# williamedwards/autompc

Measured on AMD Instinct MI355X. Metric: MPC solves/sec (MPPI, n_samples x horizon rollouts + update per solve), higher is better.
Workload: dtype f64; 1 GPU; c3: HalfCheetah (17-dim state, 6-dim ctrl), MLP 2x256, MPPI 4096 samples x 30 horizon; random-weight model, QuadCost Q=I R=0.01I F=I, sigma=1 lmda=1, 1 independent solve(s) per step per GPU, noise=device; n_samples=4096, horizon=30, state_dim=17, ctrl_dim=6, parallelism=independent solves per GPU (dp1)

## Files before the change

autompc_amd/csrc/mlp_tile.hpp:

```cpp
#pragma once
#include <hip/hip_runtime.h>

#include <type_traits>

#include "probe.hpp"

namespace ampc {

constexpr int kMaxHidden = 4;
constexpr int kMaxWaves = 8;

typedef double d4 __attribute__((ext_vector_type(4)));
typedef float f4 __attribute__((ext_vector_type(4)));

template <typename T> struct Acc;
template <> struct Acc<double> { using type = d4; };
template <> struct Acc<float> { using type = f4; };

__device__ __forceinline__ d4 mfma16(double a, double b, d4 c) {
  if constexpr (Probe::no_mfma) { c[0] += a * b; return c; }
  else return __builtin_amdgcn_mfma_f64_16x16x4f64(a, b, c, 0, 0, 0);
}
__device__ __forceinline__ f4 mfma16(float a, float b, f4 c) {
  if constexpr (Probe::no_mfma) { c[0] += a * b; return c; }
// ... 376 lines not shown
        __builtin_amdgcn_sched_group_barrier(0x020, SG, 0);
        __builtin_amdgcn_sched_group_barrier(0x100, 2 * MT, 0);
#pragma unroll
        for (int i = 0; i < SG / 2; ++i) {
          __builtin_amdgcn_sched_group_barrier(0x008, 2 * MT * NT, 0);
          __builtin_amdgcn_sched_group_barrier(0x100, MT, 0);
        }
      } else if constexpr (sizeof(T) == 4 && (Probe::f32_ahead > 0 || Probe::f32_fine > 0)) {
        constexpr int AH = Probe::f32_ahead > 0 ? Probe::f32_ahead : 2;
        __builtin_amdgcn_sched_group_barrier(0x100, AH * MT, 0);
        if constexpr (Probe::f32_fine == 1) {
#pragma unroll
          for (int i = 0; i < SG; ++i) {
            __builtin_amdgcn_sched_group_barrier(0x008, MT * NT, 0);
            if (i + AH < SG) __builtin_amdgcn_sched_group_barrier(0x100, MT, 0);
            __builtin_amdgcn_sched_group_barrier(0x020, 1, 0);
          }
        } else if constexpr (Probe::f32_fine == 2) {
          constexpr int H1 = (MT * NT + 1) / 2, H2 = MT * NT - H1;
#pragma unroll
          for (int i = 0; i < SG; ++i) {
            __builtin_amdgcn_sched_group_barrier(0x008, H1, 0);
            if (i + AH < SG) __builtin_amdgcn_sched_group_barrier(0x100, MT, 0);
            if (H2 > 0) __builtin_amdgcn_sched_group_barrier(0x008, H2, 0);
            __builtin_amdgcn_sched_group_barrier(0x020, 1, 0);
          }
        } else if constexpr (Probe::f32_fine == 3) {
#pragma unroll
          for (int i = 0; i < SG; ++i) {
            __builtin_amdgcn_sched_group_barrier(0x008, MT * NT, 0);
            __builtin_amdgcn_sched_group_barrier(0x020, 1, 0);
            if (i + AH < SG) __builtin_amdgcn_sched_group_barrier(0x100, MT, 0);
          }
        } else {
#pragma unroll
          for (int i = 0; i < SG / 2; ++i) {
            __builtin_amdgcn_sched_group_barrier(0x008, 2 * MT * NT, 0);
            if (2 * i + AH < SG) __builtin_amdgcn_sched_group_barrier(0x100, MT, 0);
            if (2 * i + AH + 1 < SG) __builtin_amdgcn_sched_group_barrier(0x100, MT, 0);
            __builtin_amdgcn_sched_group_barrier(0x020, 2, 0);
          }
        }
      } else if (REG0 && sgi < FS) {
#pragma unroll
        for (int i = 0; i < SG / 2; ++i) {
          __builtin_amdgcn_sched_group_barrier(0x008, 2 * MT * NT, 0);
          __builtin_amdgcn_sched_group_barrier(0x020, 2, 0);
        }
      } else {
        __builtin_amdgcn_sched_group_barrier(0x100, 2 * MT, 0);
#pragma unroll
        for (int i = 0; i < SG / 2; ++i) {
          __builtin_amdgcn_sched_group_barrier(0x008, 2 * MT * NT, 0);
          __builtin_amdgcn_sched_group_barrier(0x100, MT, 0);
          __builtin_amdgcn_sched_group_barrier(0x020, 2, 0);
        }
      }
    }
    if (OWN && sgi == FS - 1) {
      lds_barrier();
      mid();
    }
    if constexpr (Probe::valu_pad) {
      if (KS >= 16 && sgi >= 2 && sgi < 10) {
        int padv = lane;
#pragma unroll
        for (int pi = 0; pi < 8; ++pi) asm volatile("v_add_u32 %0, %0, 1" : "+v"(padv));
        asm volatile("" :: "v"(padv));
      }
    }
    if constexpr (Probe::valu_pad64) {
      if (KS >= 16 && sgi >= 2 && sgi < 10) {
        double padd = (double)lane;
#pragma unroll
        for (int pi = 0; pi < 8; ++pi) asm volatile("v_add_f64 %0, %0, 1.0" : "+v"(padd));
        asm volatile("" :: "v"(padd));
      }
    }
  }
}


template <typename T, int NT, int MT, int W, bool DERIV = false, int LEAN = 0, typename SH = DynShape,
          bool WIDE = false, bool PINNED = false, bool BIAS0K = false>
struct TileNet {
  using acc_t = typename Acc<T>::type;
  static constexpr int M = 16 * MT;
  static constexpr int HP = 16 * NT * W;
  static constexpr int KSH = HP / 4;
  static constexpr int KSW = KSH / W;
  static constexpr int KS0MAX = 12;
  static constexpr int GH = 8;
  static constexpr int NOMAX = WIDE ? 4 : 2;
  static constexpr bool OWN = (16 * NT == 4 * GH) && (((KSH / GH) & (KSH / GH - 1)) == 0);
  static constexpr bool PIN = PINNED && SH::kStatic && sizeof(T) == 8;
  static constexpr bool CHAIN = PIN && MT == 1 && !DERIV && !WIDE && LEAN == 0;
  static constexpr int BR = (CHAIN && W == 8) ? 4 : 1;
  static constexpr bool CHAIN_BIAS_LDS = CHAIN && BR == 1;
  static constexpr bool BIAS0_IN_K = BIAS0K && CHAIN && !Probe::no_res0 && SH::k1p <= 24 && SH::nx + SH::nu < SH::k1p;

  static constexpr int KS0RES = sizeof(T) == 4 ? KS0MAX : 6;
  T pf0[KS0RES][NT];
  __device__ __forceinline__ static bool resident0(const MlpDev<T>& m) {
    return !Probe::no_res0 && LEAN < 2 && (sizeof(T) == 4 || MT == 1) && m.k1p <= 4 * KS0RES;
  }

  __device__ __forceinline__ static unsigned slice0(const MlpDev<T>& m, int w) {
    return (unsigned)(m.W(0) - m.WB()) + (unsigned)w * (unsigned)(m.k1p / 4) * 64u * NT;
  }
  __device__ __forceinline__ static unsigned slice_h(const MlpDev<T>& m, int l, int w) {
    return (unsigned)(m.W(l) - m.WB()) + (unsigned)w * (unsigned)KSH * 64u * NT;
  }
  rsrc_t wr;
  template <int KS> __device__ __forceinline__ const T (&first0() const)[KS][NT] {
    return reinterpret_cast<const T(&)[KS][NT]>(pf0);
  }
  template <int KS> __device__ __forceinline__ T (&first0())[KS][NT] {
    return reinterpret_cast<T(&)[KS][NT]>(pf0);
  }

  static constexpr bool RESIDENT_OUT = WIDE || (LEAN < 2 && !(MT == 4 && sizeof(T) == 8));
  T wout[KSW][NOMAX];

  __device__ __forceinline__ static void load_out(const MlpDev<T>& m, int w, int lane,
                                                  T (&dst)[KSW][NOMAX]) {
    if constexpr (WIDE) {
      const int tiles = m.nxp / 16;
      const T* wl = m.W(m.n_hidden) + ((size_t)w * KSW * 64 + lane) * tiles;
#pragma unroll
      for (int ks = 0; ks < KSW; ++ks)
#pragma unroll
        for (int n = 0; n < NOMAX; ++n) dst[ks][n] = n < tiles ? wl[(size_t)ks * 64 * tiles + n] : T(0);
    } else if (m.nxp == 16) {
      const T* wl = m.W(m.n_hidden) + ((size_t)w * KSW * 64 + lane);
#pragma unroll
      for (int ks = 0; ks < KSW; ++ks) { dst[ks][0] = wl[ks * 64]; dst[ks][1] = T(0); }
    } else {
      const T* wl = m.W(m.n_hidden) + ((size_t)w * KSW * 64 + lane) * 2;
#pragma unroll
      for (int ks = 0; ks < KSW; ++ks) { const vec_t<T, 2> v = *reinterpret_cast<const vec_t<T, 2>*>(wl + ks * 128); dst[ks][0] = v[0]; dst[ks][1] = v[1]; }
      if (m.tail4) {
        const T* wt = m.WT() + ((size_t)w * KSW * 64 + lane);
#pragma unroll
        for (int ks = 0; ks < KSW; ++ks) dst[ks][1] = wt[ks * 64];
      }
    }
  }

  static constexpr bool RESIDENT_BIAS = LEAN < 1 && (MT == 1);
  static constexpr int kResBias = 2;
  T bias_r[kResBias][NT][BR];
  T pfn[GH][NT];
  ProbeWave<Probe::wave_time> probe;

  lds_ptr<const T> bq_;
  static constexpr int RS = sizeof(T) == 8 ? 4 : 1;
  static constexpr int NGH = KSH / GH;
  lds_ptr<T> ep_[2][4];
  lds_ptr<const T> rd_[2][NGH];
  lds_ptr<const T> ro_;
  lds_ptr<const T> x0_;
  lds_ptr<T> pp_, pt_;
  int w_;

  __device__ __forceinline__ void pin(const MlpDev<T>& m_in, const TileLds& L_in, T* lds) {
    if constexpr (PIN) {
      const MlpDev<T> m = SH::template fold<T>(m_in);
      const TileLds L = SH::template fold_lds<T, M, W>(L_in);
      const int lane = threadIdx.x & 63;
      const int w = w_ = __builtin_amdgcn_readfirstlane(threadIdx.x >> 6);
      const int i = lane & 15, q = lane >> 4;
      const int as = L.act_stride;
      const bool pingpong = L.act2 != L.act;
#pragma unroll
      for (int b = 0; b < 2; ++b) {
        T* buf = lds + (b ? L.act2 : L.act);
        const bool read = b == 0 ? m.n_hidden > 1 : (pingpong && m.n_hidden > 2);
        const bool written = CHAIN ? read : (b == 0 || pingpong);
#pragma unroll
        for (int r = 0; r < 4; ++r) {
          if constexpr (CHAIN)
            ep_[b][r] = (written && r == 0) ? lds_pin(buf + i * as + 16 * NT * w + q) : lds_ptr<T>(nullptr);
// ... 234 lines not shown
    };
    auto epilogue_chain = [&](int l, acc_t (&acc)[MT][NT], int db, bool store) {
      switch (m.act) {
        case 0: chain_k(l, acc, db, store, std::integral_constant<int, 0>{}); break;
        case 1: chain_k(l, acc, db, store, std::integral_constant<int, 1>{}); break;
        case 2: chain_k(l, acc, db, store, std::integral_constant<int, 2>{}); break;
        case 4: chain_k(l, acc, db, store, std::integral_constant<int, 4>{}); break;
        default: chain_k(l, acc, db, store, std::integral_constant<int, 3>{}); break;
      }
    };

    bool side_done = false;
    {
      acc_t acc[MT][NT];
#pragma unroll
      for (int mt = 0; mt < MT; ++mt)
#pragma unroll
        for (int nt = 0; nt < NT; ++nt) acc[mt][nt] = acc_t{0, 0, 0, 0};
      const unsigned wl = slice0(m, w);
      const T* A = lds + L.xu;
      if (m.n_hidden == 1) prefetch_next(1);
      if (resident0(m)) {
        const auto arow0 = [&] {
          if constexpr (PIN) return x0_;
          else return A + i * L.xu_stride + q;
        }();
        switch (m.k1p) {
          case 8: layer0_resident<2>(arow0, L.xu_stride, acc); break;
          case 16: layer0_resident<4>(arow0, L.xu_stride, acc); break;
          case 24: layer0_resident<6>(arow0, L.xu_stride, acc); break;
          default:
            if constexpr (KS0RES >= 12) {
              switch (m.k1p) {
                case 32: layer0_resident<8>(arow0, L.xu_stride, acc); break;
                case 40: layer0_resident<10>(arow0, L.xu_stride, acc); break;
                default: layer0_resident<12>(arow0, L.xu_stride, acc); break;
              }
            }
            break;
        }
      } else {
        auto layer0_streamed = [&](auto ks) {
          layer_mma_static<T, NT, MT, decltype(ks)::value, 2, false, false, 2, false, CHAIN>(
              A, L.xu_stride, wr, wl, lane, first0<2>(), acc);
        };
        switch (m.k1p) {
          case 8: layer0_streamed(std::integral_constant<int, 2>{}); break;
          case 16: layer0_streamed(std::integral_constant<int, 4>{}); break;
          case 24: layer0_streamed(std::integral_constant<int, 6>{}); break;
          case 32: layer0_streamed(std::integral_constant<int, 8>{}); break;
          case 40: layer0_streamed(std::integral_constant<int, 10>{}); break;
          case 48: layer0_streamed(std::integral_constant<int, 12>{}); break;
          default:
            if constexpr (WIDE) {
              switch (m.k1p) {
                case 56: layer0_streamed(std::integral_constant<int, 14>{}); break;
                case 64: layer0_streamed(std::integral_constant<int, 16>{}); break;
                case 72: layer0_streamed(std::integral_constant<int, 18>{}); break;
                default: layer0_streamed(std::integral_constant<int, 20>{}); break;
              }
            } else {
              layer0_streamed(std::integral_constant<int, 12>{});
            }
            break;
        }
      }
      AMPC_MARK(2);
      if constexpr (CHAIN) epilogue_chain(0, acc, 0, m.n_hidden > 1);
      else epilogue(0, acc, act, 0);
    }
    if (!OWN && m.n_hidden > 1) lds_barrier();
    AMPC_MARK(3);

    for (int l = 1; l < m.n_hidden; ++l) {
      acc_t acc[MT][NT];
#pragma unroll
      for (int mt = 0; mt < MT; ++mt)
#pragma unroll
        for (int nt = 0; nt < NT; ++nt) {
          acc[mt][nt] = acc_t{0, 0, 0, 0};
        }
      constexpr int SGH = (sizeof(T) == 8 && !Probe::sg8) ? GH / 2 : GH;
      auto mid = [&] {
        if (!Probe::side_late && l == 1) { side(); side_done = true; }
      };
      auto pinned_group = [&](int g) {
        if constexpr (OWN) return cur ? rd_[1][g] : rd_[0][g];
        else return (cur ? rd_[1][0] : rd_[0][0]) + 4 * GH * g;
      };
      if constexpr (CHAIN && OWN)
        layer_mma_static<T, NT, MT, KSH, GH, (W == 8), OWN, SGH, true, true>(
            act, as, wr, slice_h(m, l, w), lane, pfn, acc, w, mid, pinned_group,
            [&](int kk) { return own[kk >> 2][kk & 3]; });
      else if constexpr (PIN)
        layer_mma_static<T, NT, MT, KSH, GH, (W == 8), OWN, SGH, true, CHAIN>(
            act, as, wr, slice_h(m, l, w), lane, pfn, acc, w, mid, pinned_group);
      else
        layer_mma_static<T, NT, MT, KSH, GH, (W == 8), OWN, SGH, true>(
            act, as, wr, slice_h(m, l, w), lane, pfn, acc, w, mid);
      AMPC_MARK(4);
      prefetch_next(l + 1);
      const bool stores = !CHAIN || l + 1 < m.n_hidden;
      if (!pingpong && stores) lds_barrier();
      AMPC_MARK(5);
      if constexpr (CHAIN) epilogue_chain(l, acc, pingpong ? cur ^ 1 : 0, stores);
      else epilogue(l, acc, act_other, pingpong ? cur ^ 1 : 0);
      if (!OWN && l + 1 < m.n_hidden) lds_barrier();
      AMPC_MARK(6);
      { T* tmp = act; act = act_other; act_other = tmp; }
      if (pingpong) cur ^= 1;
    }

    acc_t oacc[MT][NOMAX];
    T tacc[MT];
#pragma unroll
    for (int mt = 0; mt < MT; ++mt) {
      tacc[mt] = T(0);
#pragma unroll
      for (int n = 0; n < NOMAX; ++n) oacc[mt][n] = acc_t{0, 0, 0, 0};
    }
    {
      const auto arow = [&] {
        if constexpr (PIN) return ro_;
        else return static_cast<const T*>(act) + act_row<T>(i) * as + q + 4 * w * KSW;
      }();
      auto afrag = [&](int mt, int ks) -> T {
        if constexpr (CHAIN) return own[ks >> 2][ks & 3];
        else return arow[mt * 16 * as + 4 * ks];
      };
      if constexpr (WIDE) {
#pragma unroll
        for (int ks = 0; ks < KSW; ++ks)
#pragma unroll
          for (int mt = 0; mt < MT; ++mt) {
            const T a = afrag(mt, ks);
#pragma unroll
            for (int n = 0; n < NOMAX; ++n)
              if (n < no) oacc[mt][n] = mfma16_x<kRealOut>(a, wo(ks, n), oacc[mt][n]);
          }
      } else if (no == 1) {
#pragma unroll
        for (int ks = 0; ks < KSW; ++ks)
#pragma unroll
          for (int mt = 0; mt < MT; ++mt)
            oacc[mt][0] = mfma16_x<kRealOut>(afrag(mt, ks), wo(ks, 0), oacc[mt][0]);
      } else if (m.tail4) {
#pragma unroll
        for (int ks = 0; ks < KSW; ++ks)
#pragma unroll
          for (int mt = 0; mt < MT; ++mt) {
            const T a = afrag(mt, ks);
            oacc[mt][0] = mfma16_x<kRealOut>(a, wo(ks, 0), oacc[mt][0]);
            tacc[mt] = kRealOut ? mfma4(a, wo(ks, 1), tacc[mt]) : tacc[mt] + a * wo(ks, 1);
          }
      } else {
#pragma unroll
        for (int ks = 0; ks < KSW; ++ks)
#pragma unroll
          for (int mt = 0; mt < MT; ++mt) {
            const T a = afrag(mt, ks);
            oacc[mt][0] = mfma16_x<kRealOut>(a, wo(ks, 0), oacc[mt][0]);
            oacc[mt][1] = mfma16_x<kRealOut>(a, wo(ks, 1), oacc[mt][1]);
          }
      }
    }
    AMPC_MARK(7);
    prefetch0(m);
    if (m.n_hidden > 1) prefetch_next(1);
    if (!side_done) {
      if (m.n_hidden == 1) lds_barrier();
      side();
    }
    if (L.part_alias) lds_barrier();
    AMPC_MARK(8);
    const int ps = part_stride((int)sizeof(T), m.nxp);
    T* part = lds + L.part + w * M * ps;
    const int nfull = m.tail4 ? 1 : no;
#pragma unroll
    for (int mt = 0; mt < MT; ++mt) {
#pragma unroll
      for (int n = 0; n < NOMAX; ++n)
        if (n < nfull) {
#pragma unroll
          for (int r = 0; r < 4; ++r) {
            if constexpr (PIN) {
              pp_[(16 * mt + RS * r) * ps + 16 * n] = oacc[mt][n][r];
            } else {
              const int row = 16 * mt + acc_row<T>(q, r);
              part[row * ps + 16 * n + i] = oacc[mt][n][r];
            }
          }
        }
      if (m.tail4) {
        if constexpr (PIN) pt_[16 * mt * ps] = tacc[mt];
        else part[(16 * mt + tail_row(lane)) * ps + 16 + tail_col(lane)] = tacc[mt];
      }
    }
    AMPC_MARK(13);
    lds_barrier();
    AMPC_MARK(9);
  }

  __device__ __forceinline__ static T output(const MlpDev<T>& m_in, const TileLds& L_in, const T* lds,
                                             int row, int col) {
    const MlpDev<T> m = SH::template fold<T>(m_in);
    const TileLds L = SH::template fold_lds<T, M, W>(L_in);
    const int ps = part_stride((int)sizeof(T), m.nxp);
    const T* p = lds + L.part + row * ps + col;
    T y = lds[L.bias + m.n_hidden * m.hpad + col];
#pragma unroll
    for (int w = 0; w < W; ++w) y += p[w * M * ps];
    return y;
  }
};

template <typename T>
__device__ __forceinline__ T quad_rows(const T* __restrict__ Mx, const T* __restrict__ v,
                                       const T* __restrict__ g, int n, int r, int tps, bool diag) {
  T acc = T(0);
  if (diag) {
    for (int i = r; i < n; i += tps) {
      const T d = v[i] - (g ? g[i] : T(0));
      acc += Mx[i * n + i] * d * d;
    }
  } else {
    for (int i = r; i < n; i += tps) {
      T s = T(0);
      for (int j = 0; j < n; ++j) s += Mx[i * n + j] * (v[j] - (g ? g[j] : T(0)));
      acc += (v[i] - (g ? g[i] : T(0))) * s;
    }
  }
  return acc;
}

template <typename T>
__device__ __forceinline__ T affine_rows(const T* __restrict__ lin, const T* __restrict__ v,
                                         const T* __restrict__ g, int n, int r, int tps, T c) {
  T acc = r == 0 ? c : T(0);
  for (int i = r; i < n; i += tps) acc += lin[i] * (v[i] - g[i]);
  return acc;
}

constexpr int kMaxInd = 8;
__host__ __device__ constexpr int ind_stride(int no) { return 2 * no + 2; }
template <typename T> __device__ __forceinline__ bool ind_entry(int kind, T x, T a, T b) {
  if (kind == 1) { const T d = x - a; return d > b || -d > b; }
  return x < a || x > b;
}
template <typename T> __device__ __forceinline__ bool ind_void(int kind, T x, T b) {
  return kind == 1 && x != x && b < T(INFINITY);
}
template <typename T>
__device__ __forceinline__ T indicator_rows(const T* __restrict__ tab, int n_ind, const T* __restrict__ v, int vs,
                                            int no, int r, int tps) {
  T acc = T(0);
  const int lane = threadIdx.x & 63;
  for (int k = 0; k < n_ind; ++k) {
    const T* tk = tab + (size_t)k * ind_stride(no);
    const int kind = (int)tk[0];
    bool viol = false, nan_in = false;
    for (int i = r; i < no; i += tps) {
      viol = viol || ind_entry<T>(kind, v[i * vs], tk[2 + i], tk[2 + no + i]);
      nan_in = nan_in || ind_void<T>(kind, v[i * vs], tk[2 + no + i]);
    }
    const unsigned long long bal = __ballot(viol), nal = __ballot(nan_in);
    const int sh = lane & ~(tps - 1);
    const unsigned long long msk = tps >= 64 ? ~0ull : (1ull << tps) - 1ull;
    const unsigned long long grp = tps >= 64 ? bal : (bal >> sh) & msk;
    const unsigned long long gna = tps >= 64 ? nal : (nal >> sh) & msk;
    if (r == 0 && grp != 0ull && gna == 0ull) acc += T(1);
  }
  return acc;
}
template <typename T>
__device__ __forceinline__ T indicator_all(const T* __restrict__ tab, int n_ind, const T* __restrict__ v, int vs, int no) {
  T acc = T(0);
  for (int k = 0; k < n_ind; ++k) {
    const T* tk = tab + (size_t)k * ind_stride(no);
    const int kind = (int)tk[0];
    bool viol = false, nan_in = false;
    for (int i = 0; i < no; ++i) {
      viol = viol || ind_entry<T>(kind, v[i * vs], tk[2 + i], tk[2 + no + i]);
      nan_in = nan_in || ind_void<T>(kind, v[i * vs], tk[2 + no + i]);
    }
    if (viol && !nan_in) acc += T(1);
  }
  return acc;
}

}
```

autompc_amd/csrc/mppi_kernels.hpp:

```cpp
#pragma once
#include "mlp_tile.hpp"
#include <stdint.h>

namespace ampc {

constexpr int kWG = 256;
constexpr int kWaves = 4;

template <typename T> struct MppiProblem {
  int N, H;
  int tile0;
  int cost_idx;
  T lam_over_sigma;
  T neg_inv_lambda;
  T sqrt_sigma;
  long long eps_off;
  long long epso_off;
  long long cost_off;
  int a_off;
  unsigned noise_id;
  int model;
};

template <typename T> struct MppiArgs {
// ... 29 lines not shown
  int n_ind;
  const T* ind_tab;
  const long long* model_delta;
  const int* tile_order;
  unsigned long long* done_flag;
  unsigned long long done_seq;
};

template <typename T>
__device__ __forceinline__ void publish_u(const MppiArgs<T>& args, int p, int nu, int j, T value) {
  args.u_out[p * nu + j] = value;
  if (args.done_flag) {
    __threadfence_system();
    if (j == 0) __hip_atomic_store(args.done_flag + p, args.done_seq, __ATOMIC_RELEASE, __HIP_MEMORY_SCOPE_SYSTEM);
  }
}

template <typename T> __device__ __forceinline__ T block_min(T v, T* scratch);
template <typename T> __device__ __forceinline__ T block_sum(T v, T* scratch);
template <typename T> __device__ __forceinline__ T wave_sum(T v);


template <typename T> __device__ __forceinline__ void st_agent(T* p, T v) {
  __hip_atomic_store(p, v, __ATOMIC_RELAXED, __HIP_MEMORY_SCOPE_AGENT);
}
template <typename T> __device__ __forceinline__ T ld_agent(const T* p) {
  return __hip_atomic_load(const_cast<T*>(p), __ATOMIC_RELAXED, __HIP_MEMORY_SCOPE_AGENT);
}

template <typename T, int NTHR>
__device__ __forceinline__ void finish_update_if_last(const MppiArgs<T>& args, const MppiProblem<T>& pr, int p,
                                                      int tile_m, T* scratch) {
  __shared__ int ticket_s;
  const int tid = threadIdx.x, nu = args.mlp.nu, H = pr.H;
  const int tiles = (pr.N + tile_m - 1) / tile_m;
  asm volatile("s_waitcnt vmcnt(0)" ::: "memory");
  __syncthreads();
  if (tid == 0) ticket_s = __hip_atomic_fetch_add(&args.tile_done[p], 1, __ATOMIC_RELAXED, __HIP_MEMORY_SCOPE_AGENT);
  __syncthreads();
  if (ticket_s != tiles - 1) return;
  if (tid == 0) __hip_atomic_store(&args.tile_done[p], 0, __ATOMIC_RELAXED, __HIP_MEMORY_SCOPE_AGENT);
  const T* st = args.tile_stat + 2 * (size_t)pr.tile0;
  T* sc = scratch;
  T* ss = scratch + tiles;
  T* part = ss + tiles;
  for (int i = tid; i < tiles; i += NTHR) { sc[i] = ld_agent(st + 2 * i); ss[i] = ld_agent(st + 2 * i + 1); }
  __syncthreads();
  T vmin = T(INFINITY);
  for (int i = 0; i < tiles; ++i) vmin = sc[i] < vmin ? sc[i] : vmin;
  __syncthreads();
  for (int i = tid; i < tiles; i += NTHR)
    sc[i] = (sc[i] < T(INFINITY)) ? exp(pr.neg_inv_lambda * (sc[i] - vmin)) : T(0);
  __syncthreads();
  T ssum = T(0);
  for (int i = 0; i < tiles; ++i) ssum += sc[i] * ss[i];
  const T* tp = args.tile_part + (size_t)pr.tile0 * args.hnu_stride;
  const int E = H * nu;
  for (int e0 = 0; e0 < E; e0 += NTHR) {
    const int ne = (E - e0) < NTHR ? (E - e0) : NTHR;
    const int NG = NTHR / ne;
    const int g = tid / ne, e = e0 + tid - g * ne;
    T acc = T(0);
    if (g < NG)
      for (int i = g; i < tiles; i += NG) acc += sc[i] * ld_agent(tp + (size_t)i * args.hnu_stride + e);
    __syncthreads();
    if (g < NG) part[tid] = acc;
    __syncthreads();
    if (tid < ne) {
      T tot = T(0);
      for (int k = 0; k < NG; ++k) tot += part[k * ne + tid];
      const int ee = e0 + tid, t = ee / nu, j = ee - t * nu;
      const int ts = (t + 1 < H) ? t + 1 : H - 1;
      const T a_new = args.act_in[pr.a_off + ts * nu + j] + tot / ssum;
      args.act_out[pr.a_off + ee] = a_new;
      if (t == 0) publish_u(args, p, nu, j, a_new * args.bounds[2 * nu + j]);
    }
  }
}

template <typename T, int NT, int MT, int W, typename SH = DynShape, bool WIDE = false>
__global__ __launch_bounds__(64 * W) void mppi_rollout_kernel(const MppiArgs<T> args) {
  extern __shared__ __attribute__((aligned(16))) unsigned char smem_raw[];
  T* lds = reinterpret_cast<T*>(smem_raw);
  using Net = TileNet<T, NT, MT, W, false, 0, SH, WIDE, true, true>;
  constexpr int M = 16 * MT, NTHR = 64 * W;
  constexpr int TPS = NTHR / M;
  constexpr int EPT = (16 + TPS - 1) / TPS;
  constexpr bool EXT = !SH::kStatic;
  const int tile = args.tile_order ? __builtin_amdgcn_readfirstlane(args.tile_order[blockIdx.x]) : (int)blockIdx.x;
  const int p = args.tile_prob[tile];
  const MppiProblem<T> pr = args.probs[p];
  const MlpDev<T> mlp = plan_model<SH, T>(args.mlp, [&] { return model_delta_of(args.model_delta, pr.model); });
  const TileLds L = SH::template fold_lds<T, M, W>(args.lds);
  const int tid = threadIdx.x;
  const int nx = mlp.nx, nu = mlp.nu, no = SH::kStatic ? SH::no : args.obs_dim;
  const int xs_ = L.xu_stride;
  const bool diag = args.cost_diag != 0, affine = args.cost_affine != 0;
  const int cost_stride = SH::kStatic ? cost_block_stride(SH::no, SH::nu) : args.cost_stride;
  const int lds_cost = SH::kStatic ? L.extra : args.lds_cost;
  const int lds_aseq = SH::kStatic ? round_up(L.extra + cost_stride + 3 * SH::nu, 4) : args.lds_aseq;

  const int first = (tile - pr.tile0) * M;
  const int H = pr.H, N = pr.N;

  if (W == 8) {
    if (__builtin_amdgcn_readfirstlane(threadIdx.x >> 6) < 4) __builtin_amdgcn_s_setprio(2);
    else __builtin_amdgcn_s_setprio(0);
  }
  Net net;
  net.init(mlp);
  net.pin(mlp, L, lds);

  T* aseq = lds + lds_aseq;
  T* cpar = lds + lds_cost;
  const T* Qm = cpar;
  const T* Rm = Qm + no * no;
  const T* Fm = Rm + nu * nu;
  const T* goal = Fm + no * no;
  const T* lin = goal + no;
  const T* lint = lin + no;
  const T* blo = cpar + cost_stride;
  const T* bhi = blo + nu;
  const T* bsc = bhi + nu;
  T* xu = lds + L.xu;

  tile_load_constants<T, W>(mlp, L, lds, M);
  for (int i = tid; i < cost_stride; i += NTHR)
    cpar[i] = args.costs_par[(size_t)pr.cost_idx * cost_stride + i];
  for (int i = tid; i < 3 * nu; i += NTHR) cpar[cost_stride + i] = args.bounds[i];
  for (int i = tid; i < H * nu; i += NTHR) {
    const int t = i / nu, j = i - t * nu;
    const int ts = (t + 1 < H) ? t + 1 : H - 1;
    aseq[i] = args.act_in[pr.a_off + ts * nu + j];
  }

  const int m = tid / TPS, r = tid % TPS;
  const int n = first + m;
  const bool valid = n < N;
  const T* eps_row = args.eps + pr.eps_off + (size_t)(valid ? n : 0) * H * nu;
  T* epso = args.eps_out + pr.epso_off;

  T c_part = T(0), ca_part = T(0);
  T e_next[EPT];
#pragma unroll
  for (int e = 0; e < EPT; ++e) {
    const int j = r + e * TPS;
    e_next[e] = (valid && j < nu) ? eps_row[j] : T(0);
  }
  __syncthreads();
  for (int i = tid; i < M * nx; i += NTHR) {
    const int row = i / nx, col = i - row * nx;
    xu[row * xs_ + col] = args.x0[p * nx + col];
  }
  if constexpr (Net::BIAS0_IN_K)
    for (int i = tid; i < M; i += NTHR) xu[i * xs_ + SH::k1p - 1] = T(1);

  T lo_r[EPT], hi_r[EPT], sc_r[EPT], rd_r[EPT];
  const T* eps_nx = eps_row + nu + r;
  auto actions = [&](int t) {
#pragma unroll
    for (int e = 0; e < EPT; ++e) {
      const int j = r + e * TPS;
      if (j < nu) {
        const T a = aseq[t * nu + j];
        T A = e_next[e] + a;
        A = A < lo_r[e] ? lo_r[e] : A;
        A = A > hi_r[e] ? hi_r[e] : A;
        const T ec = A - a;
        if (valid && args.write_eps_out) epso[((size_t)t * N + n) * nu + j] = ec;
        if (args.lds_eps >= 0) lds[args.lds_eps + (t * M + m) * nu + j] = ec;
        ca_part += A * ec;
        const T u = A * sc_r[e];
        xu[m * xs_ + nx + j] = u;
        if (diag) c_part += rd_r[e] * u * u;
        if constexpr (Net::PIN) {
          if (t + 1 < H && valid) e_next[e] = eps_nx[e * TPS];
        } else {
          if (t + 1 < H) e_next[e] = valid ? eps_row[(t + 1) * nu + j] : T(0);
        }
      }
    }
    if constexpr (Net::PIN) eps_nx += nu;
  };
#pragma unroll
  for (int e = 0; e < EPT; ++e) {
    const int j = r + e * TPS;
    lo_r[e] = j < nu ? blo[j] : T(0);
    hi_r[e] = j < nu ? bhi[j] : T(0);
    sc_r[e] = j < nu ? bsc[j] : T(0);
    rd_r[e] = j < nu ? Rm[j * nu + j] : T(0);
  }
  actions(0);
  __syncthreads();
  if (diag) c_part += quad_rows<T>(Qm, xu + m * xs_, goal, no, r, TPS, true);
  if (affine) {
    if (diag) c_part += affine_rows<T>(lin, xu + m * xs_, goal, no, r, TPS, T(0));
    if (r == 0) c_part += T(H) * lint[no];
  }

  AMPC_PROBE_KERNEL_BEGIN(net.probe);
  constexpr int XPT = ((WIDE ? 64 : 32) + TPS - 1) / TPS;
  T qd_r[XPT], gl_r[XPT], ql_r[XPT];
#pragma unroll
  for (int e = 0; e < XPT; ++e) {
    const int i = r + e * TPS;
    qd_r[e] = (diag && i < no) ? Qm[i * no + i] : T(0);
    gl_r[e] = i < no ? goal[i] : T(0);
    ql_r[e] = (diag && i < no) ? lin[i] : T(0);
  }
  for (int t = 0; t < H; ++t) {
    AMPC_PROBE_STEP(net.probe, t == 5);
    AMPC_MARK(0);
    if constexpr (EXT)
      if (args.n_ind) c_part += indicator_rows<T>(args.ind_tab, args.n_ind, xu + m * xs_, 1, no, r, TPS);
    if (!diag && !Probe::no_cost) {
      c_part += quad_rows<T>(Qm, xu + m * xs_, goal, no, r, TPS, false);
      c_part += quad_rows<T>(Rm, xu + m * xs_ + nx, nullptr, nu, r, TPS, false);
      if (affine) c_part += affine_rows<T>(lin, xu + m * xs_, goal, no, r, TPS, T(0));
    }
    AMPC_MARK(1);
    net.run_side(mlp, L, lds, [&] { if (t + 1 < H) actions(t + 1); });
#pragma unroll
    for (int e = 0; e < XPT; ++e) {
      const int i = r + e * TPS;
      if (i < nx) {
        const T xn = xu[m * xs_ + i] + Net::output(mlp, L, lds, m, i);
        xu[m * xs_ + i] = xn;
        if (diag && i < no && t + 1 < H) {
          const T d = xn - gl_r[e];
          c_part += (qd_r[e] * d + ql_r[e]) * d;
        }
      }
    }
    AMPC_MARK(12);
    AMPC_MARK(10);
    lds_barrier();
    AMPC_MARK(11);
  }

  AMPC_PROBE_KERNEL_END();
  T term = quad_rows<T>(Fm, xu + m * xs_, goal, no, r, TPS, diag);
  if (affine) term += affine_rows<T>(lint, xu + m * xs_, goal, no, r, TPS, lint[no + 1]);
  T c = c_part + pr.lam_over_sigma * ca_part;
  if (args.term_mode == 1) c += term;
#pragma unroll
  for (int off = TPS / 2; off > 0; off >>= 1) {
    c += __shfl_xor(c, off);
    term += __shfl_xor(term, off);
  }
  if (r == 0 && valid) {
    args.costs[pr.cost_off + n] = c;
    if (n == N - 1) args.term_last[p] = term;
  }
  if (args.lds_eps < 0) return;

  T* cred = lds + args.lds_red;
  T* sred = cred + M;
  if (r == 0) cred[m] = valid ? c : T(INFINITY);
  __syncthreads();
  T mw = cred[0];
  for (int i = 1; i < M; ++i) mw = cred[i] < mw ? cred[i] : mw;
  const bool dead_tile = !(mw < T(INFINITY));
  if (tid < M)
    sred[tid] = (first + tid < N && !dead_tile) ? exp(pr.neg_inv_lambda * (cred[tid] - mw)) : T(0);
  __syncthreads();
  const T* el = lds + args.lds_eps;
  T* tp = args.tile_part + (size_t)tile * args.hnu_stride;
  for (int e = tid; e < H * nu; e += NTHR) {
    const int t = e / nu, j = e - t * nu;
    T s = T(0);
    for (int i = 0; i < M; ++i) s += sred[i] * el[(t * M + i) * nu + j];
    tp[e] = s;
  }
  if (tid == 0) {
    T ss = T(0);
    for (int i = 0; i < M; ++i) ss += sred[i];
    args.tile_stat[2 * tile] = mw;
    args.tile_stat[2 * tile + 1] = ss;
  }
}

constexpr int kMaxNu = 16;

template <typename T>
__device__ __forceinline__ void philox_normal_pair(T* __restrict__ out, long long count, T scale, uint64_t seed,
                                                   uint64_t stream, uint32_t id, long long pair);
template <typename T> struct NoiseAhead {
  T* eps;
  unsigned long long seed, stream;
};

template <typename T>
__global__ __launch_bounds__(kWG) void mppi_combine_kernel(const MppiArgs<T> args, int tile_m,
                                                           const NoiseAhead<T> ahead) {
  __shared__ T scratch[kWaves];
  __shared__ T red[kWaves][kMaxNu + 1];
  const int p = blockIdx.y, t = blockIdx.x, tid = threadIdx.x;
  const MppiProblem<T> pr = args.probs[p];
  if (t >= args.max_h) {
    if (ahead.eps)
      philox_normal_pair<T>(ahead.eps + pr.eps_off, (long long)pr.N * pr.H * args.mlp.nu, pr.sqrt_sigma, ahead.seed,
                            ahead.stream, pr.noise_id, (long long)(t - args.max_h) * kWG + tid);
    return;
  }
  if (t >= pr.H) return;
  const int nu = args.mlp.nu, H = pr.H;
  const int tiles = (pr.N + tile_m - 1) / tile_m;
  const T* st = args.tile_stat + 2 * (size_t)pr.tile0;
  const T* tp = args.tile_part + (size_t)pr.tile0 * args.hnu_stride + t * nu;
  const bool has0 = tid < tiles;
  const int i0 = has0 ? tid : 0;
  const T m0 = st[2 * i0], s0 = st[2 * i0 + 1];
  T row0[kMaxNu];
// ... 219 lines not shown
```

autompc_amd/csrc/probe.hpp:

```cpp
#pragma once
#include <hip/hip_runtime.h>

#ifdef AMPC_X_RIC_OCC
#define AMPC_PROBE_RIC_OCC __attribute__((amdgpu_waves_per_eu(4, 4)))
#else
#define AMPC_PROBE_RIC_OCC
#endif

namespace ampc {

#define AMPC_PROBE_FLAG(name, macro) static constexpr bool name = macro
struct Probe {
#ifdef AMPC_X_NOMFMA
  AMPC_PROBE_FLAG(no_mfma, true);
#else
  AMPC_PROBE_FLAG(no_mfma, false);
#endif
#ifdef AMPC_X_NOHID
  AMPC_PROBE_FLAG(no_hid, true);
#else
  AMPC_PROBE_FLAG(no_hid, false);
#endif
#ifdef AMPC_X_NOL0
  AMPC_PROBE_FLAG(no_l0, true);
#else
  AMPC_PROBE_FLAG(no_l0, false);
#endif
#ifdef AMPC_X_NOOUT
  AMPC_PROBE_FLAG(no_out, true);
#else
  AMPC_PROBE_FLAG(no_out, false);
#endif
#ifdef AMPC_X_NOLOAD
  AMPC_PROBE_FLAG(no_load, true);
#else
  AMPC_PROBE_FLAG(no_load, false);
#endif
#ifdef AMPC_X_NOSCHED
  AMPC_PROBE_FLAG(no_sched, true);
#else
  AMPC_PROBE_FLAG(no_sched, false);
#endif
#ifdef AMPC_X_VMEMFIRST
  AMPC_PROBE_FLAG(vmem_first, true);
#else
  AMPC_PROBE_FLAG(vmem_first, false);
#endif
#ifdef AMPC_X_VALUPAD
  AMPC_PROBE_FLAG(valu_pad, true);
#else
  AMPC_PROBE_FLAG(valu_pad, false);
#endif
#ifdef AMPC_X_VALUPAD64
  AMPC_PROBE_FLAG(valu_pad64, true);
#else
  AMPC_PROBE_FLAG(valu_pad64, false);
#endif
#ifdef AMPC_X_NORES0
  AMPC_PROBE_FLAG(no_res0, true);
#else
  AMPC_PROBE_FLAG(no_res0, false);
#endif
#ifdef AMPC_X_F32AHEAD
  static constexpr int f32_ahead = AMPC_X_F32AHEAD;
#else
  static constexpr int f32_ahead = 0;
#endif
#ifdef AMPC_X_F32FINE
  static constexpr int f32_fine = AMPC_X_F32FINE;
#else
  static constexpr int f32_fine = 1;
#endif
#ifdef AMPC_X_NOJACPIPE
  AMPC_PROBE_FLAG(jac_pipe, false);
#else
  AMPC_PROBE_FLAG(jac_pipe, true);
#endif
#ifdef AMPC_X_SG8
  AMPC_PROBE_FLAG(sg8, true);
#else
  AMPC_PROBE_FLAG(sg8, false);
#endif
#ifdef AMPC_X_SIDELATE
  AMPC_PROBE_FLAG(side_late, true);
#else
  AMPC_PROBE_FLAG(side_late, false);
#endif
#ifdef AMPC_X_NOCOST
  AMPC_PROBE_FLAG(no_cost, true);
#else
  AMPC_PROBE_FLAG(no_cost, false);
#endif
#ifdef AMPC_X_LSWGLOBAL
  AMPC_PROBE_FLAG(lsw_global, true);
#else
  AMPC_PROBE_FLAG(lsw_global, false);
#endif
#ifdef AMPC_X_WAVETIME
  AMPC_PROBE_FLAG(wave_time, true);
#else
  AMPC_PROBE_FLAG(wave_time, false);
#endif
#if defined(AMPC_X_PHASETIME) && !defined(AMPC_X_WAVETIME)
  AMPC_PROBE_FLAG(phase_time, true);
#else
  AMPC_PROBE_FLAG(phase_time, false);
#endif
};
#undef AMPC_PROBE_FLAG

template <bool ON> struct ProbeWave {};
template <> struct ProbeWave<true> {
  long long m[16];
  bool on = false;
};

#if defined(AMPC_X_WAVETIME)
__device__ long long g_wave_marks[8 * 16];
#define AMPC_PROBE_LOCALS(pw) auto& _xm = (pw).m; const bool _xon = (pw).on; (void)_xm; (void)_xon
#define AMPC_MARK(idx) do { if (_xon) _xm[idx] = (long long)__builtin_amdgcn_s_memtime(); } while (0)
#define AMPC_MARK_ALWAYS(idx) do { } while (0)
#define AMPC_PROBE_KERNEL_BEGIN(pw) auto& _xm = (pw).m; _Pragma("unroll") for (int i_ = 0; i_ < 16; ++i_) _xm[i_] = 0
#define AMPC_PROBE_STEP(pw, cond) (pw).on = (blockIdx.x == 7 && (cond)); const bool _xon = (pw).on
#define AMPC_PROBE_KERNEL_END()                                                                  \
  do {                                                                                           \
    if (blockIdx.x == 7 && (threadIdx.x & 63) == 0)                                              \
      for (int i_ = 0; i_ < 16; ++i_) g_wave_marks[(threadIdx.x >> 6) * 16 + i_] = _xm[i_];      \
  } while (0)
#elif defined(AMPC_X_PHASETIME)
__device__ long long g_phase_marks[128];
#define AMPC_PROBE_LOCALS(pw) do { } while (0)
#define AMPC_MARK(idx)                                                              \
  do {                                                                              \
    if (blockIdx.x == 7 && threadIdx.x == 0 && g_phase_marks[63] == 1)              \
      g_phase_marks[idx] = (long long)__builtin_amdgcn_s_memtime();                 \
  } while (0)
#define AMPC_MARK_ALWAYS(idx)                                                       \
  do {                                                                              \
    if (blockIdx.x == 7 && threadIdx.x == 0)                                        \
      g_phase_marks[idx] = (long long)__builtin_amdgcn_s_memtime();                 \
  } while (0)
#define AMPC_PROBE_KERNEL_BEGIN(pw) do { } while (0)
#define AMPC_PROBE_STEP(pw, cond) \
  do { if (blockIdx.x == 7 && threadIdx.x == 0) g_phase_marks[63] = (cond) ? 1 : 0; } while (0)
#define AMPC_PROBE_KERNEL_END() do { } while (0)
#else
#define AMPC_PROBE_LOCALS(pw) do { } while (0)
#define AMPC_MARK(idx) do { } while (0)
#define AMPC_MARK_ALWAYS(idx) do { } while (0)
#define AMPC_PROBE_KERNEL_BEGIN(pw) do { } while (0)
#define AMPC_PROBE_STEP(pw, cond) do { } while (0)
#define AMPC_PROBE_KERNEL_END() do { } while (0)
#endif

#if defined(AMPC_X_PHASETIME) && !defined(AMPC_X_WAVETIME)
#define AMPC_LSW_MARK(pm, on, i) do { if (on) (pm)[i] = (long long)__builtin_amdgcn_s_memtime(); } while (0)
#define AMPC_LSW_DUMP(pm, w, n)                                                                   \
  do {                                                                                            \
    if (blockIdx.x == 7 && (threadIdx.x & 63) == 0)                                               \
      for (int i_ = 0; i_ < (n); ++i_) g_phase_marks[64 + (w) * 16 + i_] = (pm)[i_];              \
  } while (0)
#define AMPC_IMARK(idx) AMPC_MARK(idx)
#define AMPC_IMARK_ALWAYS(idx) AMPC_MARK_ALWAYS(idx)
#define AMPC_IPROBE_STEP(cond) AMPC_PROBE_STEP(0, cond)
#else
#define AMPC_LSW_MARK(pm, on, i) do { } while (0)
#define AMPC_LSW_DUMP(pm, w, n) do { } while (0)
#define AMPC_IMARK(idx) do { } while (0)
#define AMPC_IMARK_ALWAYS(idx) do { } while (0)
// ... 45 lines not shown
```

Before: 3513 solves/s.

## Move MPPI side action computation to tail of MLP forward pass

Adds a SIDETAIL template option to the tiled MLP and enables it in the MPPI rollout kernel. The side work (computing next-step noisy clamped actions) moves from between hidden layers to after the output partials are stored, just before the final barrier. A sched_barrier is placed where it used to run. The aim is to stop side work from interrupting the hidden-layer MFMA stream and instead hide it behind the barrier wait. An optional shadow variant, behind a probe flag, prefetches the action sequence and output partials before summing.

New measurement: 3543 solves/s, median of 6. About the same (+0.8%).

```diff
diff --git a/autompc_amd/csrc/mlp_tile.hpp b/autompc_amd/csrc/mlp_tile.hpp
--- a/autompc_amd/csrc/mlp_tile.hpp
+++ b/autompc_amd/csrc/mlp_tile.hpp
@@ -482,7 +482,7 @@
 
 
 template <typename T, int NT, int MT, int W, bool DERIV = false, int LEAN = 0, typename SH = DynShape,
-          bool WIDE = false, bool PINNED = false, bool BIAS0K = false>
+          bool WIDE = false, bool PINNED = false, bool BIAS0K = false, bool SIDETAIL = false>
 struct TileNet {
   using acc_t = typename Acc<T>::type;
   static constexpr int M = 16 * MT;
@@ -498,6 +498,7 @@
   static constexpr int BR = (CHAIN && W == 8) ? 4 : 1;
   static constexpr bool CHAIN_BIAS_LDS = CHAIN && BR == 1;
   static constexpr bool BIAS0_IN_K = BIAS0K && CHAIN && !Probe::no_res0 && SH::k1p <= 24 && SH::nx + SH::nu < SH::k1p;
+  static constexpr bool SIDE_TAIL = SIDETAIL && CHAIN && SH::n_hidden >= 2 && !Probe::side_mid;
 
   static constexpr int KS0RES = sizeof(T) == 4 ? KS0MAX : 6;
   T pf0[KS0RES][NT];
@@ -898,7 +899,8 @@
         }
       constexpr int SGH = (sizeof(T) == 8 && !Probe::sg8) ? GH / 2 : GH;
       auto mid = [&] {
-        if (!Probe::side_late && l == 1) { side(); side_done = true; }
+        if (!SIDE_TAIL && !Probe::side_late && l == 1) { side(); side_done = true; }
+        if constexpr (SIDE_TAIL) __builtin_amdgcn_sched_barrier(0);
       };
       auto pinned_group = [&](int g) {
         if constexpr (OWN) return cur ? rd_[1][g] : rd_[0][g];
@@ -983,9 +985,11 @@
     AMPC_MARK(7);
     prefetch0(m);
     if (m.n_hidden > 1) prefetch_next(1);
-    if (!side_done) {
-      if (m.n_hidden == 1) lds_barrier();
-      side();
+    if constexpr (!SIDE_TAIL) {
+      if (!side_done) {
+        if (m.n_hidden == 1) lds_barrier();
+        side();
+      }
     }
     if (L.part_alias) lds_barrier();
     AMPC_MARK(8);
@@ -1013,6 +1017,7 @@
       }
     }
     AMPC_MARK(13);
+    if constexpr (SIDE_TAIL && !Probe::side_shadow) side();
     lds_barrier();
     AMPC_MARK(9);
   }
@@ -1026,6 +1031,22 @@
     T y = lds[L.bias + m.n_hidden * m.hpad + col];
 #pragma unroll
     for (int w = 0; w < W; ++w) y += p[w * M * ps];
+    return y;
+  }
+  __device__ __forceinline__ static void output_request(const MlpDev<T>& m_in, const TileLds& L_in, const T* lds,
+                                                        int row, int col, T& yb, T (&pv)[W]) {
+    const MlpDev<T> m = SH::template fold<T>(m_in);
+    const TileLds L = SH::template fold_lds<T, M, W>(L_in);
+    const int ps = part_stride((int)sizeof(T), m.nxp);
+    const T* p = lds + L.part + row * ps + col;
+    yb = lds[L.bias + m.n_hidden * m.hpad + col];
+#pragma unroll
+    for (int w = 0; w < W; ++w) pv[w] = p[w * M * ps];
+  }
+  __device__ __forceinline__ static T output_sum(T yb, const T (&pv)[W]) {
+    T y = yb;
+#pragma unroll
+    for (int w = 0; w < W; ++w) y += pv[w];
     return y;
   }
 };
diff --git a/autompc_amd/csrc/mppi_kernels.hpp b/autompc_amd/csrc/mppi_kernels.hpp
--- a/autompc_amd/csrc/mppi_kernels.hpp
+++ b/autompc_amd/csrc/mppi_kernels.hpp
@@ -135,7 +135,7 @@
 __global__ __launch_bounds__(64 * W) void mppi_rollout_kernel(const MppiArgs<T> args) {
   extern __shared__ __attribute__((aligned(16))) unsigned char smem_raw[];
   T* lds = reinterpret_cast<T*>(smem_raw);
-  using Net = TileNet<T, NT, MT, W, false, 0, SH, WIDE, true, true>;
+  using Net = TileNet<T, NT, MT, W, false, 0, SH, WIDE, true, true, true>;
   constexpr int M = 16 * MT, NTHR = 64 * W;
   constexpr int TPS = NTHR / M;
   constexpr int EPT = (16 + TPS - 1) / TPS;
@@ -210,12 +210,12 @@
 
   T lo_r[EPT], hi_r[EPT], sc_r[EPT], rd_r[EPT];
   const T* eps_nx = eps_row + nu + r;
-  auto actions = [&](int t) {
+  auto actions = [&](int t, const T* a_pre) {
 #pragma unroll
     for (int e = 0; e < EPT; ++e) {
       const int j = r + e * TPS;
       if (j < nu) {
-        const T a = aseq[t * nu + j];
+        const T a = a_pre ? a_pre[e] : aseq[t * nu + j];
         T A = e_next[e] + a;
         A = A < lo_r[e] ? lo_r[e] : A;
         A = A > hi_r[e] ? hi_r[e] : A;
@@ -243,7 +243,7 @@
     sc_r[e] = j < nu ? bsc[j] : T(0);
     rd_r[e] = j < nu ? Rm[j * nu + j] : T(0);
   }
-  actions(0);
+  actions(0, nullptr);
   __syncthreads();
   if (diag) c_part += quad_rows<T>(Qm, xu + m * xs_, goal, no, r, TPS, true);
   if (affine) {
@@ -272,16 +272,50 @@
       if (affine) c_part += affine_rows<T>(lin, xu + m * xs_, goal, no, r, TPS, T(0));
     }
     AMPC_MARK(1);
-    net.run_side(mlp, L, lds, [&] { if (t + 1 < H) actions(t + 1); });
-#pragma unroll
-    for (int e = 0; e < XPT; ++e) {
-      const int i = r + e * TPS;
-      if (i < nx) {
-        const T xn = xu[m * xs_ + i] + Net::output(mlp, L, lds, m, i);
-        xu[m * xs_ + i] = xn;
-        if (diag && i < no && t + 1 < H) {
-          const T d = xn - gl_r[e];
-          c_part += (qd_r[e] * d + ql_r[e]) * d;
+    auto state_cost = [&](int e, int i, T xn) {
+      if (diag && i < no && t + 1 < H) {
+        const T d = xn - gl_r[e];
+        c_part += (qd_r[e] * d + ql_r[e]) * d;
+      }
+    };
+    if constexpr (!(Net::SIDE_TAIL && Probe::side_shadow)) {
+      net.run_side(mlp, L, lds, [&] { if (t + 1 < H) actions(t + 1, nullptr); });
+#pragma unroll
+      for (int e = 0; e < XPT; ++e) {
+        const int i = r + e * TPS;
+        if (i < nx) {
+          const T xn = xu[m * xs_ + i] + Net::output(mlp, L, lds, m, i);
+          xu[m * xs_ + i] = xn;
+          state_cost(e, i, xn);
+        }
+      }
+    } else {
+      net.run_side(mlp, L, lds, [] {});
+      const int a_at = (t + 1 < H ? t + 1 : H - 1) * nu;
+      T a_nx[EPT];
+#pragma unroll
+      for (int e = 0; e < EPT; ++e) {
+        const int j = r + e * TPS;
+        a_nx[e] = aseq[a_at + (j < nu ? j : 0)];
+      }
+      __builtin_amdgcn_sched_barrier(0);
+      T yb[XPT], pv[XPT][W], xo[XPT];
+#pragma unroll
+      for (int e = 0; e < XPT; ++e) {
+        const int i = r + e * TPS, ic = i < nx ? i : 0;
+        Net::output_request(mlp, L, lds, m, ic, yb[e], pv[e]);
+        xo[e] = xu[m * xs_ + ic];
+      }
+      __builtin_amdgcn_sched_barrier(0);
+      if (t + 1 < H) actions(t + 1, a_nx);
+      __builtin_amdgcn_sched_barrier(0);
+#pragma unroll
+      for (int e = 0; e < XPT; ++e) {
+        const int i = r + e * TPS;
+        if (i < nx) {
+          const T xn = xo[e] + Net::output_sum(yb[e], pv[e]);
+          xu[m * xs_ + i] = xn;
+          state_cost(e, i, xn);
         }
       }
     }
diff --git a/autompc_amd/csrc/probe.hpp b/autompc_amd/csrc/probe.hpp
--- a/autompc_amd/csrc/probe.hpp
+++ b/autompc_amd/csrc/probe.hpp
@@ -85,6 +85,16 @@
   AMPC_PROBE_FLAG(side_late, true);
 #else
   AMPC_PROBE_FLAG(side_late, false);
+#endif
+#ifdef AMPC_X_SIDEMID
+  AMPC_PROBE_FLAG(side_mid, true);
+#else
+  AMPC_PROBE_FLAG(side_mid, false);
+#endif
+#ifdef AMPC_X_SIDESHADOW
+  AMPC_PROBE_FLAG(side_shadow, true);
+#else
+  AMPC_PROBE_FLAG(side_shadow, false);
 #endif
 #ifdef AMPC_X_NOCOST
   AMPC_PROBE_FLAG(no_cost, true);
```
